# al-mcintyre/mCaller

Measured on NVIDIA B200. Metric: per-read site calls/sec, higher is better.
Workload: dtype f64

## Files before the change

mcaller_b200/csrc/records.cu:

```cuda
#include "parse.cuh"

namespace {

constexpr int SCAN_THREADS = 256;
constexpr int SCAN_IPT = 8;
constexpr int SCAN_BLOCK = SCAN_THREADS * SCAN_IPT;

__global__ void __launch_bounds__(SCAN_THREADS) k_scan_reduce(const uint32_t *__restrict__ in, int64_t n_cap,
                                                            const unsigned long long *__restrict__ d_n,
                                                            unsigned long long *__restrict__ block_sums) {
    __shared__ int s_warp[SCAN_THREADS / 32 + 1];
    const int64_t n = d_n ? mc_dev_count(d_n, n_cap) : n_cap;
    const int64_t base = (int64_t)blockIdx.x * SCAN_BLOCK;
    unsigned long long acc = 0ull;
#pragma unroll
    for (int j = 0; j < SCAN_IPT; ++j) {
        const int64_t i = base + (int64_t)j * SCAN_THREADS + threadIdx.x;
        if (i < n) acc += in[i];
    }
    for (int d = 16; d > 0; d >>= 1) acc += __shfl_down_sync(0xffffffffu, acc, d);
    __shared__ unsigned long long s_sum[SCAN_THREADS / 32];
    if ((threadIdx.x & 31) == 0) s_sum[threadIdx.x >> 5] = acc;
    __syncthreads();
    if (threadIdx.x == 0) {
        unsigned long long t = 0ull;
        for (int w = 0; w < SCAN_THREADS / 32; ++w) t += s_sum[w];
        block_sums[blockIdx.x] = t;
    }
    (void)s_warp;
}

__global__ void __launch_bounds__(1024) k_scan_sums(unsigned long long *__restrict__ block_sums, int64_t nb,
                                                   unsigned long long *__restrict__ d_total) {
    __shared__ unsigned long long s_w[33];
    __shared__ unsigned long long s_carry;
    if (threadIdx.x == 0) s_carry = 0ull;
    __syncthreads();
    const int lane = threadIdx.x & 31, wid = threadIdx.x >> 5;
    for (int64_t c0 = 0; c0 < nb; c0 += 1024) {
        const int64_t i = c0 + threadIdx.x;
        const unsigned long long v = (i < nb) ? block_sums[i] : 0ull;
        unsigned long long inc = v;
        for (int d = 1; d < 32; d <<= 1) {
            unsigned long long t = __shfl_up_sync(0xffffffffu, inc, d);
            if (lane >= d) inc += t;
        }
        if (lane == 31) s_w[wid] = inc;
        __syncthreads();
        if (wid == 0) {
            unsigned long long x = s_w[lane], xi = x;
            for (int d = 1; d < 32; d <<= 1) {
                unsigned long long t = __shfl_up_sync(0xffffffffu, xi, d);
                if (lane >= d) xi += t;
            }
            s_w[lane] = xi - x;
            if (lane == 31) s_w[32] = xi;
        }
        __syncthreads();
        const unsigned long long carry = s_carry;
        if (i < nb) block_sums[i] = carry + s_w[wid] + inc - v;
        __syncthreads();
        if (threadIdx.x == 0) s_carry = carry + s_w[32];
        __syncthreads();
    }
    if (threadIdx.x == 0 && d_total) *d_total = s_carry;
}

__global__ void __launch_bounds__(SCAN_THREADS) k_scan_down(const uint32_t *__restrict__ in, int64_t n_cap,
                                                          const unsigned long long *__restrict__ d_n,
                                                          const unsigned long long *__restrict__ block_sums,
                                                          uint32_t *__restrict__ out) {
    __shared__ int s_warp[SCAN_THREADS / 32 + 1];
    const int64_t n = d_n ? mc_dev_count(d_n, n_cap) : n_cap;
    if ((int64_t)blockIdx.x * SCAN_BLOCK >= n) return;
    const int64_t base = (int64_t)blockIdx.x * SCAN_BLOCK + (int64_t)threadIdx.x * SCAN_IPT;
    uint32_t v[SCAN_IPT];
    int sum = 0;
#pragma unroll
    for (int j = 0; j < SCAN_IPT; ++j) {
        const int64_t i = base + j;
        v[j] = (i < n) ? in[i] : 0u;
        sum += (int)v[j];
    }
    int total;
    int off = mc_block_exscan<SCAN_THREADS>(sum, s_warp, total);
    uint32_t run = (uint32_t)block_sums[blockIdx.x] + (uint32_t)off;
#pragma unroll
    for (int j = 0; j < SCAN_IPT; ++j) {
        const int64_t i = base + j;
        if (i < n) out[i] = run;
        run += v[j];
    }
}

}

int64_t mc_exscan_ws_bytes(int64_t n) { return ((n + SCAN_BLOCK - 1) / SCAN_BLOCK + 1) * 8 + 256; }

int mc_exscan_u32(const uint32_t *d_in, uint32_t *d_out, int64_t n_cap, const uint64_t *d_n, uint64_t *d_total, void *d_ws,
                  cudaStream_t st) {
    if (n_cap <= 0) {
        if (d_total) MC_CUDA_CHECK(cudaMemsetAsync(d_total, 0, 8, st));
        return MC_OK;
    }
    const int64_t nb = (n_cap + SCAN_BLOCK - 1) / SCAN_BLOCK;
    unsigned long long *sums = reinterpret_cast<unsigned long long *>(d_ws);
    const unsigned long long *dn = reinterpret_cast<const unsigned long long *>(d_n);
    k_scan_reduce<<<(unsigned)nb, SCAN_THREADS, 0, st>>>(d_in, n_cap, dn, sums);
    MC_LAUNCH_CHECK();
    k_scan_sums<<<1, 1024, 0, st>>>(sums, nb, reinterpret_cast<unsigned long long *>(d_total));
    MC_LAUNCH_CHECK();
    k_scan_down<<<(unsigned)nb, SCAN_THREADS, 0, st>>>(d_in, n_cap, dn, sums, d_out);
    MC_LAUNCH_CHECK();
    return MC_OK;
}

extern "C" int64_t mc_windows_workspace_bytes(int64_t rec_cap);
extern "C" int64_t mc_workspace_bytes(int64_t n) {
    if (n < 1) n = 1;
    const int64_t a = ((n * 4 + 255) / 256) * 256;
    const int64_t mine = 2 * a + mc_exscan_ws_bytes(n) + 512;
    const int64_t win = mc_windows_workspace_bytes(n);
    return mine > win ? mine : win;
}
static inline uint32_t *ws_a(void *ws) { return reinterpret_cast<uint32_t *>(ws); }
static inline uint32_t *ws_b(void *ws, int64_t n) { return reinterpret_cast<uint32_t *>(reinterpret_cast<uint8_t *>(ws) + ((n * 4 + 255) / 256) * 256); }
static inline void *ws_s(void *ws, int64_t n) { return reinterpret_cast<uint8_t *>(ws) + 2 * (((n * 4 + 255) / 256) * 256); }

namespace {

__global__ void __launch_bounds__(256) k_run_resolve(uint32_t *__restrict__ run_tab, int64_t n_runs, uint32_t *__restrict__ cnt_clean,
                                                    const unsigned long long *__restrict__ scan_counters, unsigned long long rec_in_cap) {
    const int64_t r = (int64_t)blockIdx.x * blockDim.x + threadIdx.x;
    if (r >= n_runs) return;
    if (scan_counters && (scan_counters[MC_C_OVERFLOW] != 0ull || scan_counters[MC_C_RECORDS] > rec_in_cap)) {
        cnt_clean[r] = 0u;
        return;
    }
    uint32_t count = run_tab[2 * r];
    const uint32_t v = run_tab[2 * r + 1];
    if (v & 1u) {
        int64_t p = r - 1;
        uint32_t st = 0u;
        while (p >= 0 && (st = (run_tab[2 * p + 1] >> 1) & 3u) == 0u) --p;
        if (p >= 0 && st == 1u && count > 0u) {
            run_tab[2 * r + 1] = v | 0x80000000u;
            --count;
        }
    }
    cnt_clean[r] = count;
}

__global__ void __launch_bounds__(256, 4) k_gather_finish(const uint8_t *__restrict__ text, int64_t limit, mc_refindex R,
                                                      const uint32_t *__restrict__ tile_tab, const uint32_t *__restrict__ run_tab,
                                                      const uint32_t *__restrict__ run_dst, int64_t n_tiles, int64_t n_runs, int run_len,
                                                      const mc_record *__restrict__ in, unsigned long long in_cap, mc_record *__restrict__ out,
                                                      unsigned long long out_cap, uint32_t *__restrict__ seg_flags,
                                                      uint32_t *__restrict__ run_first) {
    const int lane = threadIdx.x & 31;
    const int64_t warp0 = ((int64_t)blockIdx.x * blockDim.x + threadIdx.x) >> 5, n_warps = ((int64_t)gridDim.x * blockDim.x) >> 5;
    for (int64_t run = warp0; run < n_runs; run += n_warps) {
    const uint32_t rv = __ldg(run_tab + 2 * run + 1);
    const bool empty_run = __ldg(run_dst + run) == __ldg(run_dst + run + 1);
    if (run_first && lane == 0) run_first[run] = empty_run ? 0xFFFFFFFFu : __ldg(run_dst + run);
    if (__ldg(run_tab + 2 * run) == 0u) continue;
    const bool drop = (rv >> 31) != 0u;
    unsigned long long d_run = __ldg(run_dst + run);
    const int64_t c0 = run * run_len, c1 = min(c0 + (int64_t)run_len, n_tiles);
    long long carry_line = -1;
    uint32_t carry_span = 0u;
    for (int64_t cb = c0; cb < c1; cb += 32) {
        const int64_t c = cb + lane;
        unsigned long long src = 0ull;
        uint32_t cnt = 0u;
        if (c < c1) {
            const uint2 e = __ldg(reinterpret_cast<const uint2 *>(tile_tab) + c);
            src = e.x;
            cnt = e.y & 0xFFFFu;
            if (drop && ((e.y >> 16) & 1u) && cnt > 0u) { src += 1ull; --cnt; }
        }
        uint32_t incl = cnt;
#pragma unroll
        for (int d = 1; d < 32; d <<= 1) {
            const uint32_t t = __shfl_up_sync(0xffffffffu, incl, d);
            if (lane >= d) incl += t;
        }
        const uint32_t excl = incl - cnt, tot = __shfl_sync(0xffffffffu, incl, 31);
        for (uint32_t k0 = 0; k0 < tot; k0 += 32) {
            const uint32_t idx = k0 + lane;
            const bool act = idx < tot;
            int lo = 0, hi = 31;
#pragma unroll
            for (int st = 0; st < 5; ++st) {
                const int mid = (lo + hi + 1) >> 1;
                const uint32_t e_mid = __shfl_sync(0xffffffffu, excl, mid);
                if (e_mid <= idx) lo = mid; else hi = mid - 1;
            }
            const unsigned long long s_own = __shfl_sync(0xffffffffu, src, lo);
            const uint32_t e_own = __shfl_sync(0xffffffffu, excl, lo);
            const unsigned long long slot = s_own + (idx - e_own), dst = d_run + idx;
            const bool ok = act && slot < in_cap && dst < out_cap;
            alignas(16) mc_record r;
            long long line = -1;
            uint32_t span = 0u;
            if (ok) {
                const uint4 *sp = reinterpret_cast<const uint4 *>(in + slot);
                uint4 *dr = reinterpret_cast<uint4 *>(&r);
                dr[0] = __ldg(sp);
                dr[1] = __ldg(sp + 1);
                if (r.flags & MC_RF_RAW) mc_finish_record_win(text, limit, r);
                if (r.flags & MC_RF_CAND) {
                    const int cid = r.contig;
                    if (r.pos < __ldg(R.d_len + cid)) {
                        const int64_t g = __ldg(R.d_base + cid) + r.pos;
                        r.kbits_fwd = (uint8_t)mc_kmer_bits(R.d_site_fwd, g, R.k);
                        r.kbits_rev = (uint8_t)mc_kmer_bits(R.d_site_rev, g, R.k);
                    }
                }
                line = mc_rec_line(r);
                span = (uint32_t)r.name_off | ((uint32_t)r.name_len << 16);
            }
            long long pl = __shfl_up_sync(0xffffffffu, line, 1);
            uint32_t ps = __shfl_up_sync(0xffffffffu, span, 1);
            if (lane == 0) { pl = carry_line; ps = carry_span; }
            if (ok) {
                uint32_t sf = 1u;
                if (pl >= 0) {
                    uint32_t fl = r.flags | MC_RF_SEGKNOWN;
                    sf = 0u;
                    if ((ps >> 16) != r.name_len || bytes_differ(text + pl + (ps & 0xFFFFu), text + line + r.name_off, r.name_len)) {
                        fl |= MC_RF_NEWREAD;
                        sf = 1u;
                    }
                    r.flags = (uint8_t)fl;
                }
                if (seg_flags) seg_flags[dst] = sf;
                uint4 *dp = reinterpret_cast<uint4 *>(out + dst);
                const uint4 *sr = reinterpret_cast<const uint4 *>(&r);
                dp[0] = sr[0];
                dp[1] = sr[1];
            }
            const int last = (int)min(tot - k0, 32u) - 1;
            carry_line = __shfl_sync(0xffffffffu, line, last);
            carry_span = __shfl_sync(0xffffffffu, span, last);
        }
        d_run += tot;
    }
    }
}

__global__ void __launch_bounds__(256) k_seg_flags(const uint8_t *__restrict__ text, mc_record *__restrict__ rec, int64_t n_cap,
                                                  const unsigned long long *__restrict__ d_n, uint32_t *__restrict__ flags,
                                                  const uint32_t *__restrict__ known) {
    const int64_t n = mc_dev_count(d_n, n_cap);
    const int64_t i = (int64_t)blockIdx.x * blockDim.x + threadIdx.x;
    if (i >= n) return;
    if (known) {
        const uint32_t kf = known[i];
        if (kf < 2u) { flags[i] = kf; return; }
    }
    uint32_t f = 1u;
    const mc_record b = rec[i];
    if (b.flags & MC_RF_SEGKNOWN) {
        f = (b.flags & MC_RF_NEWREAD) ? 1u : 0u;
    } else {
        if (i > 0) {
            const mc_record a = rec[i - 1];
            if (a.name_len == b.name_len)
                f = bytes_differ(text + mc_rec_line(a) + a.name_off, text + mc_rec_line(b) + b.name_off, a.name_len) ? 1u : 0u;
        }
        rec[i].flags = (uint8_t)(b.flags | MC_RF_SEGKNOWN | (f ? MC_RF_NEWREAD : 0u));
    }
    flags[i] = f;
}

__global__ void __launch_bounds__(256) k_seg_fix(const uint8_t *__restrict__ text, mc_record *__restrict__ rec, const unsigned long long *__restrict__ d_n,
                                                int64_t n_cap, const uint32_t *__restrict__ run_first, int64_t n_runs, uint32_t *__restrict__ flags) {
    const int64_t run = (int64_t)blockIdx.x * blockDim.x + threadIdx.x;
    if (run >= n_runs) return;
    const uint32_t i = run_first[run];
    if (i == 0xFFFFFFFFu || (int64_t)i >= mc_dev_count(d_n, n_cap)) return;
    uint32_t f = 1u;
    const mc_record b = rec[i];
    if (i > 0u) {
        const mc_record a = rec[i - 1];
        if (a.name_len == b.name_len)
            f = bytes_differ(text + mc_rec_line(a) + a.name_off, text + mc_rec_line(b) + b.name_off, a.name_len) ? 1u : 0u;
    }
    rec[i].flags = (uint8_t)(b.flags | MC_RF_SEGKNOWN | (f ? MC_RF_NEWREAD : 0u));
    flags[i] = f;
}

__global__ void __launch_bounds__(256) k_seg_starts(const uint32_t *__restrict__ flags, const uint32_t *__restrict__ excl, int64_t n_cap,
                                                   const unsigned long long *__restrict__ d_n, uint32_t *__restrict__ seg_start,
                                                   const unsigned long long *__restrict__ d_nseg) {
    const int64_t n = mc_dev_count(d_n, n_cap);
    const int64_t i = (int64_t)blockIdx.x * blockDim.x + threadIdx.x;
    if (i < n && flags[i]) seg_start[excl[i]] = (uint32_t)i;
    if (i == 0) seg_start[*d_nseg] = (uint32_t)n;
}

__global__ void __launch_bounds__(256) k_seg_quality(const uint8_t *__restrict__ text, const mc_record *__restrict__ rec,
                                                    const uint32_t *__restrict__ seg_start, int64_t seg_cap,
                                                    const unsigned long long *__restrict__ d_nseg,
                                                    const mc_qual_entry *__restrict__ table, unsigned long long mask,
                                                    double *__restrict__ seg_qual, unsigned long long *__restrict__ d_err) {
    const int64_t n_seg = mc_dev_count(d_nseg, seg_cap);
    const int64_t s = (int64_t)blockIdx.x * blockDim.x + threadIdx.x;
    if (s >= n_seg) return;
    const mc_record r = rec[seg_start[s]];
    const mc_read_key key = mc_read_key_of(text + mc_rec_line(r) + r.name_off, r.name_len);
    double q = __longlong_as_double(0x7ff8000000000000ll);
    unsigned long long slot = key.hash & mask;
    for (unsigned long long probe = 0; probe <= mask; ++probe) {
        const mc_qual_entry e = table[slot];
        if (e.hash == 0ull) break;
        if (e.hash == key.hash && e.check == key.check && e.len == key.len) { q = e.qual; break; }
        slot = (slot + 1) & mask;
    }
    if (q != q) atomicAdd(d_err, 1ull);
    seg_qual[s] = q;
}

}

extern "C" int mc_order_records(const uint8_t *d_text, int64_t nbytes, const mc_refindex *ref, const uint32_t *d_tile_tab, int64_t n_tiles,
                                uint32_t *d_run_tab, int run_len, const mc_record *d_rec_in, int64_t rec_in_cap,
                                const uint64_t *d_scan_counters, mc_record *d_rec_out, int64_t rec_out_cap, uint64_t *d_n_out,
                                uint32_t *d_seg_flags, uint32_t *d_run_first, void *d_ws, void *stream) {
    MC_REQUIRE(!d_seg_flags == !d_run_first, "d_seg_flags and d_run_first go together");
    MC_REQUIRE(d_text && ref && d_tile_tab && d_run_tab && d_rec_in && d_rec_out && d_n_out && d_ws, "null pointer");
    MC_REQUIRE(run_len >= 1, "run length must be >= 1");
    cudaStream_t st = (cudaStream_t)stream;
    if (n_tiles <= 0) {
        MC_CUDA_CHECK(cudaMemsetAsync(d_n_out, 0, 8, st));
        return MC_OK;
    }
    const int64_t n_runs = (n_tiles + run_len - 1) / run_len;
    uint32_t *cnt = ws_a(d_ws), *dst = ws_b(d_ws, n_runs + 1);
    MC_CUDA_CHECK(cudaMemsetAsync(cnt + n_runs, 0, 4, st));
    k_run_resolve<<<(unsigned)((n_runs + 255) / 256), 256, 0, st>>>(d_run_tab, n_runs, cnt, reinterpret_cast<const unsigned long long *>(d_scan_counters),
                                                                   (unsigned long long)rec_in_cap);
    MC_LAUNCH_CHECK();
    int rc = mc_exscan_u32(cnt, dst, n_runs + 1, nullptr, d_n_out, ws_s(d_ws, n_runs + 1), st);
    if (rc) return rc;
    int64_t gf_blocks = (n_runs * 32 + 255) / 256;
    {
        int dev = 0, sms = 0;
        MC_CUDA_CHECK(cudaGetDevice(&dev));
        MC_CUDA_CHECK(cudaDeviceGetAttribute(&sms, cudaDevAttrMultiProcessorCount, dev));
        const int64_t resident = (int64_t)sms * 4;
        if (gf_blocks > resident) gf_blocks = resident;
    }
    k_gather_finish<<<(unsigned)gf_blocks, 256, 0, st>>>(d_text, nbytes + MC_TEXT_PAD - 64, *ref, d_tile_tab, d_run_tab, dst, n_tiles,
                                                                          n_runs, run_len, d_rec_in, (unsigned long long)rec_in_cap, d_rec_out,
                                                                          (unsigned long long)rec_out_cap, d_seg_flags, d_run_first);
    MC_LAUNCH_CHECK();
    return MC_OK;
}

extern "C" int mc_segment_reads(const uint8_t *d_text, mc_record *d_rec, const uint64_t *d_n_records, int64_t rec_cap,
                                uint32_t *d_seg_flags, const uint32_t *d_run_first, int64_t n_runs, uint32_t *d_seg_start, uint64_t *d_nseg,
                                void *d_ws, void *stream) {
    MC_REQUIRE(d_text && d_rec && d_n_records && d_seg_start && d_nseg && d_ws, "null pointer");
    cudaStream_t st = (cudaStream_t)stream;
    if (rec_cap <= 0) {
        MC_CUDA_CHECK(cudaMemsetAsync(d_nseg, 0, 8, st));
        MC_CUDA_CHECK(cudaMemsetAsync(d_seg_start, 0, 4, st));
        return MC_OK;
    }
    uint32_t *flags = ws_a(d_ws), *excl = ws_b(d_ws, rec_cap);
    const unsigned nb = (unsigned)((rec_cap + 255) / 256);
    const unsigned long long *dn = reinterpret_cast<const unsigned long long *>(d_n_records);
    if (d_seg_flags && d_run_first) {
        flags = d_seg_flags;
        if (n_runs > 0) k_seg_fix<<<(unsigned)((n_runs + 255) / 256), 256, 0, st>>>(d_text, d_rec, dn, rec_cap, d_run_first, n_runs, flags);
    } else {
        k_seg_flags<<<nb, 256, 0, st>>>(d_text, d_rec, rec_cap, dn, flags, nullptr);
    }
    MC_LAUNCH_CHECK();
    int rc = mc_exscan_u32(flags, excl, rec_cap, d_n_records, d_nseg, ws_s(d_ws, rec_cap), st);
    if (rc) return rc;
    k_seg_starts<<<nb, 256, 0, st>>>(flags, excl, rec_cap, dn, d_seg_start, reinterpret_cast<const unsigned long long *>(d_nseg));
    MC_LAUNCH_CHECK();
    return MC_OK;
}

extern "C" int mc_segment_quality(const uint8_t *d_text, const mc_record *d_rec, const uint32_t *d_seg_start, const uint64_t *d_nseg,
                                  int64_t seg_cap, const mc_qual_entry *d_table, int64_t table_size, double *d_seg_qual,
                                  uint64_t *d_err, void *stream) {
    MC_REQUIRE(d_text && d_rec && d_seg_start && d_nseg && d_table && d_seg_qual && d_err, "null pointer");
    MC_REQUIRE(table_size > 0 && (table_size & (table_size - 1)) == 0, "table size must be a power of two");
    if (seg_cap <= 0) return MC_OK;
    k_seg_quality<<<(unsigned)((seg_cap + 255) / 256), 256, 0, (cudaStream_t)stream>>>(
        d_text, d_rec, d_seg_start, seg_cap, reinterpret_cast<const unsigned long long *>(d_nseg), d_table,
        (unsigned long long)(table_size - 1), d_seg_qual, reinterpret_cast<unsigned long long *>(d_err));
    MC_LAUNCH_CHECK();
    return MC_OK;
}
```

Baseline: 49.55 million.

## Software-pipeline tile and record loads in gather-finish kernel with shared-memory prefix search

The gather-finish kernel now processes 128 tile entries per warp iteration (4 per lane) instead of 32. It stages source offsets and exclusive prefixes in per-warp shared memory and replaces the shuffle-based binary search with a shared-memory search. It prefetches the next group's tile entries, including those for the next run, and double-buffers the 32-byte record loads so the next batch is fetched while the current one is finished. The launch-bounds minimum CTAs and the grid cap drop from 4 to 3 per SM to leave room for the extra registers and shared memory, at some cost in occupancy.

```diff
diff --git a/mcaller_b200/csrc/records.cu b/mcaller_b200/csrc/records.cu
--- a/mcaller_b200/csrc/records.cu
+++ b/mcaller_b200/csrc/records.cu
@@ -151,63 +151,104 @@
     cnt_clean[r] = count;
 }
 
-__global__ void __launch_bounds__(256, 4) k_gather_finish(const uint8_t *__restrict__ text, int64_t limit, mc_refindex R,
+#ifndef MC_GF_MIN_CTAS
+#define MC_GF_MIN_CTAS 3
+#endif
+constexpr int GF_THREADS = 256, GF_MIN_CTAS = MC_GF_MIN_CTAS, GF_EPL = 4;
+__global__ void __launch_bounds__(GF_THREADS, GF_MIN_CTAS) k_gather_finish(const uint8_t *__restrict__ text, int64_t limit, mc_refindex R,
                                                       const uint32_t *__restrict__ tile_tab, const uint32_t *__restrict__ run_tab,
                                                       const uint32_t *__restrict__ run_dst, int64_t n_tiles, int64_t n_runs, int run_len,
                                                       const mc_record *__restrict__ in, unsigned long long in_cap, mc_record *__restrict__ out,
                                                       unsigned long long out_cap, uint32_t *__restrict__ seg_flags,
                                                       uint32_t *__restrict__ run_first) {
     const int lane = threadIdx.x & 31;
+    constexpr int GROUP = 32 * GF_EPL;
+    __shared__ uint32_t s_src[GF_THREADS / 32][GROUP], s_pre[GF_THREADS / 32][GROUP];
     const int64_t warp0 = ((int64_t)blockIdx.x * blockDim.x + threadIdx.x) >> 5, n_warps = ((int64_t)gridDim.x * blockDim.x) >> 5;
+    uint2 ent[GF_EPL];
+    auto load_group = [&](int64_t cb, int64_t c1) {
+#pragma unroll
+        for (int q = 0; q < GF_EPL; ++q) {
+            const int64_t c = cb + GF_EPL * lane + q;
+            ent[q] = c < c1 ? __ldg(reinterpret_cast<const uint2 *>(tile_tab) + c) : make_uint2(0u, 0u);
+        }
+    };
+    if (warp0 < n_runs) load_group(warp0 * run_len, min(warp0 * run_len + (int64_t)run_len, n_tiles));
     for (int64_t run = warp0; run < n_runs; run += n_warps) {
-    const uint32_t rv = __ldg(run_tab + 2 * run + 1);
-    const bool empty_run = __ldg(run_dst + run) == __ldg(run_dst + run + 1);
-    if (run_first && lane == 0) run_first[run] = empty_run ? 0xFFFFFFFFu : __ldg(run_dst + run);
-    if (__ldg(run_tab + 2 * run) == 0u) continue;
+    const uint32_t rv = __ldg(run_tab + 2 * run + 1), rcnt = __ldg(run_tab + 2 * run);
+    const uint32_t dst0 = __ldg(run_dst + run), dst1 = __ldg(run_dst + run + 1);
+    const bool empty_run = dst0 == dst1;
+    if (run_first && lane == 0) run_first[run] = empty_run ? 0xFFFFFFFFu : dst0;
+    const int64_t c0 = run * run_len, c1 = min(c0 + (int64_t)run_len, n_tiles);
+    const int64_t next_run = run + n_warps;
+    if (rcnt == 0u) {
+        if (next_run < n_runs) load_group(next_run * run_len, min(next_run * run_len + (int64_t)run_len, n_tiles));
+        continue;
+    }
     const bool drop = (rv >> 31) != 0u;
-    unsigned long long d_run = __ldg(run_dst + run);
-    const int64_t c0 = run * run_len, c1 = min(c0 + (int64_t)run_len, n_tiles);
+    unsigned long long d_run = dst0;
     long long carry_line = -1;
     uint32_t carry_span = 0u;
-    for (int64_t cb = c0; cb < c1; cb += 32) {
-        const int64_t c = cb + lane;
-        unsigned long long src = 0ull;
-        uint32_t cnt = 0u;
-        if (c < c1) {
-            const uint2 e = __ldg(reinterpret_cast<const uint2 *>(tile_tab) + c);
-            src = e.x;
-            cnt = e.y & 0xFFFFu;
-            if (drop && ((e.y >> 16) & 1u) && cnt > 0u) { src += 1ull; --cnt; }
-        }
-        uint32_t incl = cnt;
+    for (int64_t cb = c0; cb < c1; cb += GROUP) {
+        uint32_t *const g_src = s_src[threadIdx.x >> 5], *const g_pre = s_pre[threadIdx.x >> 5];
+        uint32_t cnt[GF_EPL], lsum = 0u;
+        __syncwarp();
+#pragma unroll
+        for (int q = 0; q < GF_EPL; ++q) {
+            uint32_t sq = ent[q].x;
+            cnt[q] = ent[q].y & 0xFFFFu;
+            if (drop && ((ent[q].y >> 16) & 1u) && cnt[q] > 0u) { sq += 1u; --cnt[q]; }
+            g_src[GF_EPL * lane + q] = sq;
+            lsum += cnt[q];
+        }
+        if (cb + GROUP < c1) load_group(cb + GROUP, c1);
+        else if (next_run < n_runs) load_group(next_run * run_len, min(next_run * run_len + (int64_t)run_len, n_tiles));
+        uint32_t incl = lsum;
 #pragma unroll
         for (int d = 1; d < 32; d <<= 1) {
             const uint32_t t = __shfl_up_sync(0xffffffffu, incl, d);
             if (lane >= d) incl += t;
         }
-        const uint32_t excl = incl - cnt, tot = __shfl_sync(0xffffffffu, incl, 31);
+        const uint32_t tot = __shfl_sync(0xffffffffu, incl, 31);
+        {
+            uint32_t e = incl - lsum;
+#pragma unroll
+            for (int q = 0; q < GF_EPL; ++q) {
+                g_pre[GF_EPL * lane + q] = e;
+                e += cnt[q];
+            }
+        }
+        __syncwarp();
+        uint4 nx0 = make_uint4(0u, 0u, 0u, 0u), nx1 = nx0;
+        bool nx_ok = false;
+        auto fetch = [&](uint32_t k0) {
+            const uint32_t idx = k0 + lane;
+            int lo = 0;
+#pragma unroll
+            for (int h = GROUP / 2; h > 0; h >>= 1)
+                if (g_pre[lo + h] <= idx) lo += h;
+            const unsigned long long slot = (unsigned long long)g_src[lo] + (idx - g_pre[lo]), dst = d_run + idx;
+            nx_ok = idx < tot && slot < in_cap && dst < out_cap;
+            if (nx_ok) {
+                const uint4 *sp = reinterpret_cast<const uint4 *>(in + slot);
+                nx0 = __ldg(sp);
+                nx1 = __ldg(sp + 1);
+            }
+        };
+        fetch(0u);
         for (uint32_t k0 = 0; k0 < tot; k0 += 32) {
-            const uint32_t idx = k0 + lane;
-            const bool act = idx < tot;
-            int lo = 0, hi = 31;
-#pragma unroll
-            for (int st = 0; st < 5; ++st) {
-                const int mid = (lo + hi + 1) >> 1;
-                const uint32_t e_mid = __shfl_sync(0xffffffffu, excl, mid);
-                if (e_mid <= idx) lo = mid; else hi = mid - 1;
-            }
-            const unsigned long long s_own = __shfl_sync(0xffffffffu, src, lo);
-            const uint32_t e_own = __shfl_sync(0xffffffffu, excl, lo);
-            const unsigned long long slot = s_own + (idx - e_own), dst = d_run + idx;
-            const bool ok = act && slot < in_cap && dst < out_cap;
+            const unsigned long long dst = d_run + k0 + lane;
+            const bool ok = nx_ok;
             alignas(16) mc_record r;
+            {
+                uint4 *dr = reinterpret_cast<uint4 *>(&r);
+                dr[0] = nx0;
+                dr[1] = nx1;
+            }
+            if (k0 + 32u < tot) fetch(k0 + 32u);
             long long line = -1;
             uint32_t span = 0u;
             if (ok) {
-                const uint4 *sp = reinterpret_cast<const uint4 *>(in + slot);
-                uint4 *dr = reinterpret_cast<uint4 *>(&r);
-                dr[0] = __ldg(sp);
-                dr[1] = __ldg(sp + 1);
                 if (r.flags & MC_RF_RAW) mc_finish_record_win(text, limit, r);
                 if (r.flags & MC_RF_CAND) {
                     const int cid = r.contig;
@@ -344,15 +385,15 @@
     MC_LAUNCH_CHECK();
     int rc = mc_exscan_u32(cnt, dst, n_runs + 1, nullptr, d_n_out, ws_s(d_ws, n_runs + 1), st);
     if (rc) return rc;
-    int64_t gf_blocks = (n_runs * 32 + 255) / 256;
+    int64_t gf_blocks = (n_runs * 32 + GF_THREADS - 1) / GF_THREADS;
     {
         int dev = 0, sms = 0;
         MC_CUDA_CHECK(cudaGetDevice(&dev));
         MC_CUDA_CHECK(cudaDeviceGetAttribute(&sms, cudaDevAttrMultiProcessorCount, dev));
-        const int64_t resident = (int64_t)sms * 4;
+        const int64_t resident = (int64_t)sms * GF_MIN_CTAS;
         if (gf_blocks > resident) gf_blocks = resident;
     }
-    k_gather_finish<<<(unsigned)gf_blocks, 256, 0, st>>>(d_text, nbytes + MC_TEXT_PAD - 64, *ref, d_tile_tab, d_run_tab, dst, n_tiles,
+    k_gather_finish<<<(unsigned)gf_blocks, GF_THREADS, 0, st>>>(d_text, nbytes + MC_TEXT_PAD - 64, *ref, d_tile_tab, d_run_tab, dst, n_tiles,
                                                                           n_runs, run_len, d_rec_in, (unsigned long long)rec_in_cap, d_rec_out,
                                                                           (unsigned long long)rec_out_cap, d_seg_flags, d_run_first);
     MC_LAUNCH_CHECK();
```

Result: no change. 49.82 million (median of 6 runs) (+0.5%).
